# nikhilTkur/Multigrid_Nikhil_C-

Hardware: AMD Instinct MI355X
Metric: fine_grid_stencil_updates_per_sec (higher is better)
Workload: dtype f64

## Files before the change

### multigrid_nikhil_c-_amd/csrc/mgx.hip

```cpp

#include "../../include/mgx.h"
#include "mgx_bottom.hpp"
#include "mgx_kernels.hpp"
#include "mgx_launch.hpp"
#include "mgx_var.hpp"
#include "mgx_krylov.hpp"
#include "mgx_dist_plan.hpp"

#include <chrono>
#include <unistd.h>
#include <cmath>
#include <cstdio>
#include <cstdlib>
#include <cstring>
#include <string>
#include <vector>

namespace {

using namespace mgx;

thread_local std::string g_create_error;

void log_runtime_libs(const char* where)
// ... 181 lines not shown
void free_level(Level& l)
{
    for (void** p : {&l.u, &l.b, &l.tmp, &l.r, &l.coef[0], &l.coef[1], &l.coef[2], &l.coef[3], &l.coef[4],
                     &l.jac[0], &l.jac[1], &l.jac[2], &l.jac[3], &l.jac[4]}) {
        if (*p) (void)hipFree(*p);
        *p = nullptr;
    }
}

int ensure_r(mgx_solver* s, Level& l)
{
    if (l.r) return MGX_OK;
    if (hipMalloc(&l.r, l.bytes) != hipSuccess) return s->fail(MGX_ERR_ALLOC, "hipMalloc failed for residual array");
    HIPCHK(s, hipMemsetAsync(l.r, 0, l.bytes, s->stream));
    return MGX_OK;
}

bool level_ok(const mgx_solver* s, int level)
{
    return level >= s->cfg.coarsest_level && level <= s->cfg.finest_level;
}

int copy_in(mgx_solver* s, Level& l, void* dst_grid, const void* src, size_t count)
{
    const size_t n = (size_t)l.N - 1;
    if (count != n * n) return s->fail(MGX_ERR_INVALID, "vector length must be n*n with n = 2^level - 1");
    const size_t es = l.esize();
    char* d = reinterpret_cast<char*>(dst_grid) + ((size_t)l.pitch + 1) * es;
    HIPCHK(s, hipMemcpy2DAsync(d, (size_t)l.pitch * es, src, n * es, n * es, n, hipMemcpyHostToDevice, s->stream));
    HIPCHK(s, hipStreamSynchronize(s->stream));
    return MGX_OK;
}

int copy_out(mgx_solver* s, Level& l, const void* src_grid, void* dst, size_t count)
{
    const size_t n = (size_t)l.N - 1;
    if (count != n * n) return s->fail(MGX_ERR_INVALID, "vector length must be n*n with n = 2^level - 1");
    const size_t es = l.esize();
    const char* p = reinterpret_cast<const char*>(src_grid) + ((size_t)l.pitch + 1) * es;
    HIPCHK(s, hipMemcpy2DAsync(dst, n * es, p, (size_t)l.pitch * es, n * es, n, hipMemcpyDeviceToHost, s->stream));
    HIPCHK(s, hipStreamSynchronize(s->stream));
    return MGX_OK;
}

inline bool tile_level(const mgx_solver* s, const Level& l) { return s->fuse.tile_max_n > 0 && l.N <= s->fuse.tile_max_n; }

void smooth_t(mgx_solver* s, Level& l, int mu)
{
    with_kernel_set(l.f64, s->cfg.smoother, s->fuse.arith, [&](auto k) {
        using K = decltype(k);
        using T = typename K::T;
        int parity = 0, launches = 0;
        if (tile_level(s, l) && smooth_tiled<T, K::SM, K::AR>((T*)l.u, (const T*)l.b, (T*)l.tmp, l.N, l.pitch, mu, s->cfg.omega,
                                                              s->fuse.tile_k, FoldArgs(), false, 0, false, s->stream, &launches) >= 0)
            parity = launches & 1;
        else
            (void)smooth_block<T>(s->cfg.smoother, (T*)l.u, (const T*)l.b, (T*)l.tmp, l.N, l.pitch, l.rows, 1, l.N, mu,
                                  s->cfg.omega, false, 1, l.N, 0, s->rows_per_chunk, s->fuse, s->stream, &parity, &launches);
        s->last_smooth_launches = launches;
        if (parity) std::swap(l.u, l.tmp);
    });
}

int var_alloc_level(mgx_solver* s, Level& l)
{
    for (void** p : {&l.coef[0], &l.coef[1], &l.coef[2], &l.coef[3], &l.coef[4], &l.jac[0], &l.jac[1], &l.jac[2], &l.jac[3], &l.jac[4]}) {
        if (hipMalloc(p, l.bytes) != hipSuccess) return s->fail(MGX_ERR_ALLOC, "hipMalloc failed for the operator's coefficient arrays");
        HIPCHK(s, hipMemsetAsync(*p, 0, l.bytes, s->stream));
    }
    return MGX_OK;
}

template <typename T>
int var_build_t(mgx_solver* s, Level& l)
{
    const dim3 blk(256), grd((l.N + 1 + 255) / 256, l.N + 1);
    hipLaunchKernelGGL((k_var_build_jacobi<T>), grd, blk, 0, s->stream, (const T*)l.coef[0], (const T*)l.coef[1], (const T*)l.coef[2],
                       (const T*)l.coef[3], (const T*)l.coef[4], (T*)l.jac[0], (T*)l.jac[1], (T*)l.jac[2], (T*)l.jac[3], (T*)l.jac[4],
                       l.N, l.pitch, (T)s->cfg.omega);
    if (l.L == s->cfg.coarsest_level && s->cfg.bottom == MGX_BOTTOM_EXACT) {
        const int n = l.N - 1, NN = n * n;
        hipLaunchKernelGGL((k_var_dense_fill<T>), dim3((NN + 255) / 256, NN), dim3(256), 0, s->stream, s->var_M, s->var_inv,
                           (const T*)l.coef[0], (const T*)l.coef[1], (const T*)l.coef[2], (const T*)l.coef[3], (const T*)l.coef[4], n, l.pitch);
        for (int k = 0; k < NN; ++k) {
            hipLaunchKernelGGL(k_gj_prow, dim3((NN + 255) / 256), dim3(256), 0, s->stream, s->var_M, s->var_inv, s->var_pm, s->var_pi, NN, k);
            hipLaunchKernelGGL(k_gj_elim, dim3(NN), dim3(256), 0, s->stream, s->var_M, s->var_inv, s->var_pm, s->var_pi, NN, k);
        }
    }
    HIPCHK(s, hipGetLastError());
    HIPCHK(s, hipStreamSynchronize(s->stream));
    l.stencil_set = true;
    for (auto& g : s->graphs) if (g.exec) (void)hipGraphExecDestroy(g.exec);
    s->graphs.clear();
    return MGX_OK;
}
int var_build(mgx_solver* s, Level& l) { return l.f64 ? var_build_t<double>(s, l) : var_build_t<float>(s, l); }

int var_ready(mgx_solver* s, int lo, int hi)
{
    if (!s->var) return MGX_OK;
    for (int l = lo; l <= hi; ++l)
        if (!s->lv[l].stencil_set)
            return s->fail(MGX_ERR_STATE, "operator of level " + std::to_string(l) + " not set (mgx_set_stencil / mgx_set_coefficient)");
    return MGX_OK;
}

template <typename T>
// ... 64 lines not shown
    const int smax = std::max(1, kcap / per);
    std::vector<double> best(mu + 1, 1e300);
    std::vector<int> pick(mu + 1, 1);
    best[0] = 0.0;
    for (int m = 1; m <= mu; ++m)
        for (int k = 1; k <= std::min(m, smax); ++k) {
            const double c = fold_pass_cost(per * k, smoother, N, post, f64, f.arith);
            if (c < 0.0) continue;
            if (k == mu && m == mu && !cycle_k_supported(per * k, rbgs, f64, post, pre, f.arith)) continue;
            const double t = best[m - k] + c + 1e-3;
            if (t < best[m] - 1e-12) { best[m] = t; pick[m] = k; }
        }
    int n = 0;
    for (int m = mu; m > 0; m -= pick[m]) parts[n++] = pick[m];
    std::sort(parts, parts + n, [](int a, int b) { return a > b; });
    return n;
}

template <typename T, int SM, int AR>
int fold_block(const FuseCfg& fc, long tile_points, const mgx_slab* f, T* u, const T* b, T* tmp, int row_lo, int row_hi,
               int mu, double omega, const mgx_slab* c, const T* coarse_e, T* coarse_b, T* coarse_zero, int crow_lo,
               int crow_hi, int restrict_mode, int zero_in, int post, double* partial, hipStream_t st, int* flips)
{
    constexpr bool rbgs = (SM == 1);
    constexpr int per = rbgs ? 2 : 1;
    const bool pre = (coarse_e != nullptr);
    const int N = 1 << f->level;
    const long pitch = level_pitch(f->level, f->dtype);
    const int first = 1 - f->row0, last = N - f->row0;
    const JacobiCoef<T> jc = jacobi_coef<T>(omega);
    FoldArgs fa;
    fa.restrict_mode = restrict_mode;
    fa.partial = partial;
    fa.win.row_first = std::max(f->row0, 0);
    fa.win.row_last = std::min(f->row0 + f->rows - 1, N);
    fa.win.crow_first = 0; fa.win.crow_last = -1; fa.win.emit_lo = 0; fa.win.emit_hi = 0;
    if (c) {
        fa.cpitch = level_pitch(c->level, c->dtype);
        fa.win.crow_first = std::max(c->row0, 0);
        fa.win.crow_last = std::min(c->row0 + c->rows - 1, N / 2);
        fa.win.emit_lo = std::max(c->row0 + crow_lo, 1);
        fa.win.emit_hi = std::min(c->row0 + crow_hi, N / 2);
        const long cback = (long)c->row0 * fa.cpitch;
        if (coarse_e) fa.coarse_e = coarse_e - cback;
        if (coarse_b) fa.coarse_b = coarse_b - cback;
        if (coarse_zero) fa.coarse_zero = coarse_zero - cback;
    }
    const long back = (long)f->row0 * pitch;
    {
        const int lo = std::max(std::max(row_lo, first), 1), hi = std::min(std::min(row_hi, last), f->rows - 1);
        const bool whole = row_lo <= first && row_hi >= last;
        if (fc.tile_max_n > 0 && hi > lo && (long)(hi - lo) * N <= tile_points && (per * mu <= fc.tile_k || whole)) {
            fa.row_lo = lo + f->row0; fa.row_hi = hi + f->row0;
            return smooth_tiled<T, SM, AR>(u - back, b - back, tmp - back, N, pitch, mu, omega, fc.tile_k, fa, pre, post,
                                           zero_in != 0, st, flips);
        }
    }
    int parts[64];
    const int np = fold_plan(fc, rbgs ? MGX_SMOOTHER_RBGS : MGX_SMOOTHER_JACOBI, N, sizeof(T) == 8, mu, pre, post, parts);
    const int rpc = env_int("MGX_ROWS", 0);
    T* src = u; T* dst = tmp;
    int done = 0, blocks = 0;
    for (int p = 0; p < np; ++p) {
        const int sw = parts[p], K = per * sw;
        const bool P = pre && p == 0;
        const int Q = (p == np - 1) ? post : 0;
        fa.zero_in = (p == 0 && zero_in) ? 1 : 0;
        const int ext = per * (mu - (done + sw)) + (p != np - 1 ? (post == 2 ? 1 : (post == 1 ? 2 : 0)) : 0);
        const int lo = std::max(std::max(row_lo - ext, first), 1), hi = std::min(std::min(row_hi + ext, last), f->rows - 1);
        if (hi > lo) {
            const int R = fuse_rows(fc, N, K, sizeof(T) == 8, hi - lo);
            if (P || Q) {
                if (!cycle_k_supported(K, rbgs, sizeof(T) == 8, Q, P, AR)) return -1;
                fa.row_lo = lo + f->row0; fa.row_hi = hi + f->row0;
                const int Rc = fuse_rows_auto(fc, N, K, sizeof(T) == 8) ? -R : R;
                const int rc = with_stages(P, Q, [&](auto s) {
                    using S = decltype(s);
                    if constexpr (S::PRE || S::POST)
                        return launch_cycle<T, S::PRE, S::POST, SM, AR>(K, src - back, b - back, dst - back, fa, N, pitch, jc.c0, jc.c1, Rc, st);
                    else
                        return -1;
                });
                if (rc < 0) return -1;
                if (Q == 2) blocks = rc;
            } else if (!rbgs && K == 1) {
                if (fa.zero_in) return -1;
                if (launch_jacobi<T>(src, b, dst, N, pitch, lo, hi, omega, rpc, st, f->rows, AR)) return -1;
            } else if (!launch_fused<T, SM, AR>(K, src, b, dst, N, pitch, lo, hi, jc.c0, jc.c1, first - 1, last, f->row0 & 1, R, st, f->rows, fa.zero_in)) {
                return -1;
            }
        }
        std::swap(src, dst);
        done += sw;
    }
    *flips = np;
    return blocks;
}

bool fold_eligible(const mgx_solver* s, const Level& l, int mu, bool pre = false, int post = 1)
{
    if (!s->fold || mu < 1 || mu > 64) return false;
    if (s->var || (post == 1 && s->cfg.restrict_mode >= MGX_RESTRICT_INJECT)) return false;
    if (tile_level(s, l)) return true;
    if (l.N < s->fuse.min_n) return false;
    const bool rbgs = (s->cfg.smoother == MGX_SMOOTHER_RBGS);
    const int per = rbgs ? 2 : 1;
    if (s->fuse.kmax < per) return false;
    int parts[64];
// ... 1551 lines not shown
```

### multigrid_nikhil_c-_amd/csrc/mgx_geom.hpp

```cpp
#pragma once

#if defined(__HIPCC__)
#define MGX_GEOM_HD __host__ __device__ __forceinline__
#else
#define MGX_GEOM_HD inline
#endif

namespace mgx {

constexpr int kGeomWavesPerBlock = 4;
constexpr int kGeomCusPerXcd = 32;
constexpr int kGeomResidentBlocks = 512;

struct CycleGeom {
    int R, Re, Rl;
    int Rf;
    int chunks, chunks_e;
    int row_last0;
    int RB, n_tall, n_short;
    long waves;
    int blocks;
};

struct CTile { int strip, r0, r1; bool active; };
// ... 175 lines not shown
        const int mid = row_last0 - (row_lo + rf);
        if (mid < rb) continue;
        const int nt_max = (8 * slots - 7 - n_edge) / si, ns_max = (8 * slots - 7) / si;
        if (nt_max < 1 || ns_max < 1) continue;
        if ((long)nt_max * ra + (long)ns_max * rb < mid) continue;
        if (rb < kn.pair_min_rows) return false;
        int nt = (int)((double)mid * ((double)nt_max * ra / ((double)nt_max * ra + (double)ns_max * rb)) / ra + 0.5);
        if (nt > nt_max) nt = nt_max;
        while (nt > 0 && (long)nt * ra > mid - rb) --nt;
        int ns = nt > 0 ? (mid - nt * ra + rb - 1) / rb : ns_max + 1;
        while (ns > ns_max && nt < nt_max && (long)(nt + 1) * ra <= mid - rb) { ++nt; ns = (mid - nt * ra + rb - 1) / rb; }
        if (nt < 1 || ns > ns_max) continue;
        const int pf = (n_edge + nt * si + 7) / 8, ps = (ns * si + 7) / 8;
        if (pf > slots || ps > slots) continue;
        CycleGeom g;
        g.R = ra; g.Re = re; g.Rl = rl; g.Rf = rf; g.RB = rb; g.n_tall = nt; g.n_short = ns;
        g.chunks_e = chunks_e; g.row_last0 = row_last0; g.chunks = 3 + nt + ns;
        g.waves = (long)g.chunks * si + 2L * chunks_e;
        g.blocks = geom_blocks(g, strips);
        if (g.blocks > kGeomResidentBlocks) continue;
        *out = g;
        return true;
    }
    return false;
}

inline CycleGeom cycle_geom_pick(int row_lo, int row_hi, int strips, int extra, int trip, int R, bool auto_rows, bool deep,
                                 const GeomKnobs& kn, bool top_edge = true, bool bot_edge = true)
{
    if (R & 1) ++R;
    R = trip_rows(R, extra, trip, 2);
    CycleGeom g = cycle_geom(row_lo, row_hi, strips, R, R, R);
    if (!deep) return g;
    auto shaped = [&](int r) {
        return cycle_geom(row_lo, row_hi, strips, r, kn.edge_short ? edge_rows_pct(r, extra, trip, kn.edge_pct) : r,
                          (kn.edge_short && bot_edge) ? edge_rows_pct(r, extra, trip, kn.last_pct) : r,
                          (kn.edge_short && top_edge) ? edge_rows_pct(r, extra, trip, kn.edge_pct) : r);
    };
    if (!auto_rows) return kn.edge_short ? shaped(R) : g;
    if (kn.pair && kn.edge_short && strips >= 3) {
        CycleGeom p;
        if (cycle_geom_paired(row_lo, row_hi, strips, extra, trip, kn, top_edge, bot_edge, &p)) return p;
    }
    bool found = false;
    for (int m = (row_hi - row_lo >= kn.min_rounds_rows ? kn.min_rounds : 1); m <= 64 && !found; ++m) {
        for (int r = trip_rows(kn.min_chunk, extra, trip, 2); r <= 204; r += trip) {
            const CycleGeom c = shaped(r);
            if (c.waves <= 2048L * m && c.blocks <= kGeomResidentBlocks * m) { g = c; found = true; break; }
        }
    }
    return g;
}

}
```

### multigrid_nikhil_c-_amd/csrc/mgx_inst.hip

```cpp
#include "mgx_launch.hpp"

namespace mgx {
using T_ = MGX_INST_T;
#if MGX_INST_KIND == 1
#if MGX_INST_PP == 0
#define PP_ 1, 2
#elif MGX_INST_PP == 1
#define PP_ 1, 0
#elif MGX_INST_PP == 2
#define PP_ 0, 1
#elif MGX_INST_PP == 3
#define PP_ 0, 2
#else
#define PP_ 1, 1
#endif
template int launch_cycle<T_, PP_, MGX_INST_SM, MGX_INST_AR>(int, const T_*, const T_*, T_*, const FoldArgs&, int, long, T_, T_, int, hipStream_t);
#elif MGX_INST_KIND == 2
template bool launch_fused<T_, MGX_INST_SM, MGX_INST_AR>(int, const T_*, const T_*, T_*, int, long, int, int, T_, T_, int, int, int, int, hipStream_t, int, int);
#elif MGX_INST_KIND == 3
template int smooth_tiled<T_, MGX_INST_SM, MGX_INST_AR>(T_*, const T_*, T_*, int, long, int, double, int, FoldArgs, bool, int, bool, hipStream_t, int*);
#else
#error "MGX_INST_KIND must be 1, 2 or 3"
#endif
}
```

### multigrid_nikhil_c-_amd/csrc/mgx_kernels.hpp

```cpp
#pragma once

#include <hip/hip_runtime.h>
#include "mgx_geom.hpp"
#include <stdint.h>
#include <type_traits>

namespace mgx {

template <int B, int E, typename F> __device__ __forceinline__ void static_for(F&& f)
{
    if constexpr (B < E) {
        f(std::integral_constant<int, B>{});
        static_for<B + 1, E>(f);
    }
}

constexpr int kWave = 64;
constexpr int kBlock = 256;
constexpr int kWavesPerBlock = kBlock / kWave;
constexpr int kOutLanes = kWave - 2;

template <typename T> struct VecOf;
template <> struct VecOf<double> { using type = double2; static constexpr int W = 2; };
template <> struct VecOf<float>  { using type = float4;  static constexpr int W = 4; };
// ... 1400 lines not shown
        double acc = 0.0;
        T prev = up;
#pragma unroll
        for (int i = 0; i < RW; ++i) {
            const T cur = u[i];
            const T below = (i == RW - 1) ? dn : u[i + 1];
            const int y = y0 + i, gy = gy0 + i;
            const T l = from_left(cur), r = from_right(cur);
            T rr = (T)0;
            if (colunk && gy > 0 && gy < N) rr = b[i] - (-nbr(prev, l, r, below) + (T)4 * cur);
            res[i] = rr;
            if (POST == 2 && y >= He && y < He + TH && gy >= row_lo && gy < row_hi && colout) acc += (double)rr * (double)rr;
            prev = cur;
        }
        if (POST == 2) {
            for (int off = 32; off > 0; off >>= 1) acc += __shfl_down(acc, off, kWave);
            if (lane == 0) wsum[wv] = acc;
            __syncthreads();
            if (threadIdx.x == 0) {
                double sum = 0.0;
                for (int w2 = 0; w2 < kWavesPerBlock; ++w2) sum += wsum[w2];
                partial[blockIdx.x] = sum;
            }
        }
        if (POST == 1) {
            T rup, rdn;
            halo_rows(res, rup, rdn);
            const int J = gx >> 1;
            const bool cst = colout && (gx & 1) == 0 && J >= 1 && J < NC;
#pragma unroll
            for (int i = 0; i < RW; ++i) {
                const T c = res[i];
                const T n = (i == 0) ? rup : res[i - 1];
                const T s2 = (i == RW - 1) ? rdn : res[i + 1];
                const int y = y0 + i, gy = gy0 + i;
                T corners = from_left(n) + from_right(n);
                corners = corners + from_left(s2);
                corners = corners + from_right(s2);
                T edges = from_left(c) + from_right(c);
                edges = edges + n;
                edges = edges + s2;
                const T o = wgt * ((corners + (T)2 * edges) + (T)4 * c);
                if (cst && y >= He && y < He + TH && (gy & 1) == 0 && gy < N && gy >= row_lo && gy < row_hi &&
                    (gy >> 1) >= win.emit_lo && (gy >> 1) < win.emit_hi) {
                    const long at = (long)(gy >> 1) * cpitch + J;
                    coarse_b[at] = o;
                    if (coarse_zero) coarse_zero[at] = (T)0;
                }
            }
        }
    }
}

static __global__ void __launch_bounds__(kBlock)
k_axpy_f32_to_f64(double* __restrict__ u, const float* __restrict__ e, double scale, int N, long pitch, long epitch,
                  int row_lo, int row_hi, int R, int strips, int chunks, int assign)
{
    const Tile t = wave_tile(strips, chunks);
    if (!t.active) return;
    const Cols c = lane_cols<2>(t.strip, N, pitch);
    const int r0 = row_lo + t.chunk * R;
    const int r1 = min(r0 + R, row_hi);
    for (int r = r0; r < r1; ++r) {
        if (c.st) {
            const float2 ev = *reinterpret_cast<const float2*>(e + (long)r * epitch + c.col);
            double2* pu = reinterpret_cast<double2*>(u + (long)r * pitch + c.col);
            double2 o = assign ? make_double2(0.0, 0.0) : *pu;
            o.x = o.x + scale * (double)ev.x;
            o.y = o.y + scale * (double)ev.y;
            if (c.col == 0) o.x = 0.0;
            *pu = o;
        }
    }
}

static __global__ void __launch_bounds__(kBlock)
k_update_residual(const double* __restrict__ u, const float* __restrict__ e, const double* __restrict__ rhs,
                  double* __restrict__ unew, float* __restrict__ r32, double scale, double inv_scale,
                  double* __restrict__ partial, int N, long pitch, long epitch, int row_lo, int row_hi,
                  int R, int strips, int chunks)
{
    __shared__ double wsum[kWavesPerBlock];
    const Tile t = wave_tile(strips, chunks);
    double acc = 0.0;
    if (t.active) {
        const Cols c = lane_cols<2>(t.strip, N, pitch);
        const int r0 = row_lo + t.chunk * R;
        const int r1 = min(r0 + R, row_hi);
        auto updated = [&](int r) {
            double2 o = make_double2(0.0, 0.0);
            if (c.ld) {
                const double2 uv = *reinterpret_cast<const double2*>(u + (long)r * pitch + c.col);
                const float2 ev = *reinterpret_cast<const float2*>(e + (long)r * epitch + c.col);
                o.x = uv.x + scale * (double)ev.x;
                o.y = uv.y + scale * (double)ev.y;
                if (c.col == 0) o.x = 0.0;
            }
            return o;
        };
        double2 up = updated(r0 - 1);
        double2 cur = updated(r0);
        for (int r = r0; r < r1; ++r) {
            const double2 dn = updated(r + 1);
            const double2 bb = vload<double2>(rhs + (long)r * pitch + c.col, c.ld);
            double2 o = residual_vec(up, cur, dn, bb);
            mask_cols(o, c.col, N);
// ... 64 lines not shown
```

### multigrid_nikhil_c-_amd/csrc/mgx_launch.hpp

```cpp
#pragma once

#include "../../include/mgx.h"
#include "mgx_kernels.hpp"

#include <algorithm>
#include <cstdlib>
#include <vector>

namespace mgx {

inline long level_pitch(int level, int dtype)
{
    const long N = 1L << level;
    const long align = (dtype == MGX_DTYPE_F64) ? 32 : 64;
    return (N + 1 + align - 1) / align * align;
}

inline int env_int(const char* name, int dflt)
{
    const char* s = getenv(name);
    return (s && *s) ? atoi(s) : dflt;
}

struct FuseCfg {
    int kmax; int rows; int min_n; int fold_kmax; int fold_kmax_big; int tile_max_n; int tile_k; int fold_kmax_nopost;
    int plan_pre[8] = {0}; int n_pre = 0; int plan_post[8] = {0}; int n_post = 0; int plan_min_n = 8192;
    int arith = 0;
};

template <typename T> struct JacobiCoef { T c0, c1; };
template <typename T>
JacobiCoef<T> jacobi_coef(double omega)
{
    const T om = (T)omega;
    return {(T)(1.0 - (double)om), (T)((double)om / 4.0)};
}

template <typename T_, int SM_, int AR_> struct KernelSet { using T = T_; static constexpr int SM = SM_, AR = AR_; };
template <typename F>
decltype(auto) with_kernel_set(bool f64, int smoother, int arith, F&& f)
{
    const bool rbgs = (smoother == MGX_SMOOTHER_RBGS);
    if (f64) return rbgs ? f(KernelSet<double, 1, 0>{}) : (arith ? f(KernelSet<double, 0, 1>{}) : f(KernelSet<double, 0, 0>{}));
    return rbgs ? f(KernelSet<float, 1, 0>{}) : (arith ? f(KernelSet<float, 0, 1>{}) : f(KernelSet<float, 0, 0>{}));
}

template <typename T>
int launch_jacobi(const T* vin, const T* b, T* vout, int N, long pitch, int row_lo, int row_hi,
                  double omega, int rpc, hipStream_t st, int rows_alloc, int arith = 0)
{
    if (row_hi <= row_lo) return MGX_OK;
    if (row_lo < 1 || row_hi > rows_alloc - 1) return MGX_ERR_INVALID;
    const auto [c0, c1] = jacobi_coef<T>(omega);
    if (rpc <= 0) {
        const Launch g = make_launch(N, VecOf<T>::W, row_hi - row_lo, 1);
        if (arith) hipLaunchKernelGGL((k_jacobi_rows<T, 1>), dim3(g.blocks), dim3(kBlock), 0, st, vin, b, vout, N, pitch,
                                      row_lo, row_hi, g.strips, c0, c1, rows_alloc);
        else hipLaunchKernelGGL((k_jacobi_rows<T, 0>), dim3(g.blocks), dim3(kBlock), 0, st, vin, b, vout, N, pitch,
                                row_lo, row_hi, g.strips, c0, c1, rows_alloc);
        return MGX_OK;
    }
    const Launch g = make_launch(N, VecOf<T>::W, row_hi - row_lo, rpc);
    if (arith) hipLaunchKernelGGL((k_jacobi<T, 1>), dim3(g.blocks), dim3(kBlock), 0, st, vin, b, vout, N, pitch,
                                  row_lo, row_hi, g.R, g.strips, g.chunks, c0, c1, rows_alloc);
    else hipLaunchKernelGGL((k_jacobi<T, 0>), dim3(g.blocks), dim3(kBlock), 0, st, vin, b, vout, N, pitch,
                            row_lo, row_hi, g.R, g.strips, g.chunks, c0, c1, rows_alloc);
    return MGX_OK;
}

template <typename T>
void launch_rbgs(const T* vin, const T* b, T* vout, int N, long pitch, int row_lo, int row_hi,
                 int row_parity, int bnd_lo, int bnd_hi, int rpc, hipStream_t st)
{
    if (row_hi <= row_lo) return;
    const Launch g = make_launch(N, VecOf<T>::W, row_hi - row_lo, rpc);
    hipLaunchKernelGGL((k_rbgs<T>), dim3(g.blocks), dim3(kBlock), 0, st, vin, b, vout, N, pitch,
                       row_lo, row_hi, g.R, g.strips, g.chunks, row_parity, bnd_lo, bnd_hi);
}
// ... 32 lines not shown
        }
    }
    return false;
}

inline int fuse_rows_deep(int N, int rows)
{
    const int strips = (N / 2 + 51) / 52;
    const int cpr = std::max(1, 2048 / strips);
    for (int m = 1; m <= 64; ++m) {
        const int R = (rows + m * cpr - 1) / (m * cpr);
        if (R <= 200) return std::max(R, 16);
    }
    return 64;
}

inline bool fuse_rows_auto(const FuseCfg& fc, int N, int K, bool f64)
{
    return fc.rows <= 0 && K >= (f64 ? 8 : 10) && N >= 2048;
}

inline int shallow_big_n() { static const int n = env_int("MGX_SHALLOW_BIG_N", 8192); return n; }
inline int shallow_mid_rows() { static const int r = env_int("MGX_SHALLOW_ROWS_MID", 48); return r; }

inline int fuse_rows(const FuseCfg& fc, int N, int K, bool f64 = true, int rows = 0)
{
    if (fc.rows > 0) return fc.rows;
    if (K <= 2) {
        static const int big2 = env_int("MGX_SHALLOW2_ROWS_BIG", 96);
        return N >= shallow_big_n() ? big2 : (N >= 4096 ? shallow_mid_rows() : 8);
    }
    if (K <= 4) {
        static const int big = env_int("MGX_SHALLOW_ROWS_BIG", 96);
        return N >= shallow_big_n() ? big : (N >= 4096 ? shallow_mid_rows() : 16);
    }
    if (f64 && K >= 8 && N >= 2048) return fuse_rows_deep(N, rows > 0 ? rows : N - 1);
    int R = N / 128;
    if (R < 8) R = 8;
    if (R > (f64 ? 64 : 32)) R = f64 ? 64 : 32;
    return R;
}

inline FuseCfg fuse_cfg()
{
    FuseCfg f;
    f.kmax = env_int("MGX_FUSE", 10);
    if (f.kmax < 1) f.kmax = 1;
    if (f.kmax > 10) f.kmax = 10;
    f.rows = env_int("MGX_FUSE_ROWS", 0);
    if (f.rows < 0) f.rows = 0;
    f.min_n = std::max(64, env_int("MGX_FUSE_MIN_N", 256));
    f.fold_kmax = std::max(1, std::min(f.kmax, env_int("MGX_FOLD_KMAX", 10)));
    f.fold_kmax_big = std::max(1, std::min(f.kmax, env_int("MGX_FOLD_KMAX_BIG", 10)));
    f.tile_max_n = std::max(0, env_int("MGX_TILE_MAX_N", 1024));
    f.tile_k = std::max(2, std::min(10, env_int("MGX_TILE_K", 10)));
    f.fold_kmax_nopost = std::max(1, std::min(f.kmax, env_int("MGX_FOLD_KMAX_NOPOST", 10)));
    auto parse = [](const char* name, int* out) {
        const char* v = std::getenv(name);
        int n = 0;
        while (v && *v && n < 8) {
            char* end = nullptr;
            const long k = std::strtol(v, &end, 10);
            if (end == v || k < 1 || k > 10) return 0;
            out[n++] = (int)k;
            v = (*end == ',') ? end + 1 : end;
            if (*end && *end != ',') return 0;
        }
        return n;
    };
    f.n_pre = parse("MGX_PLAN_PRE", f.plan_pre);
    f.n_post = parse("MGX_PLAN_POST", f.plan_post);
    f.plan_min_n = env_int("MGX_PLAN_MIN_N", 8192);
    return f;
}

constexpr double kFuseRate64[11] = {0, 1.00, 1.80, 2.45, 3.16, 3.81, 4.80, 0, 5.60, 0, 5.63};
constexpr double kFuseRate32[11] = {0, 1.00, 1.67, 2.38, 3.10, 3.77, 4.26, 0, 4.98, 0, 4.67};
constexpr double kFuseRateGS64[11] = {0, 1.00, 1.81, 2.50, 3.19, 3.12, 0, 0, 0, 0, 0};
constexpr double kFuseRateGS32[11] = {0, 1.00, 1.79, 2.20, 2.87, 2.69, 0, 0, 0, 0, 0};

inline int plan_fusion(int mu, int kmax, bool f64, int* parts, bool rbgs = false)
{
    const double* rate = rbgs ? (f64 ? kFuseRateGS64 : kFuseRateGS32) : (f64 ? kFuseRate64 : kFuseRate32);
    const int per = rbgs ? 2 : 1;
    const int smax = std::max(1, std::min(kmax, 10) / per);
    std::vector<double> best(mu + 1, 1e300);
    std::vector<int> pick(mu + 1, 1);
    best[0] = 0.0;
    for (int m = 1; m <= mu; ++m)
        for (int k = 1; k <= std::min(m, smax); ++k) {
            if (rate[k] <= 0.0) continue;
            const double c = best[m - k] + (double)k / rate[k] + 0.02;
            if (c < best[m]) { best[m] = c; pick[m] = k; }
        }
    int n = 0;
    for (int m = mu; m > 0; m -= pick[m]) parts[n++] = pick[m];
    return n;
}

template <typename T>
int smooth_block(int smoother, T* a, const T* rhs, T* b2, int N, long pitch, int rows_alloc, int row_lo, int row_hi,
                 int mu, double omega, bool shrink, int first, int last, int row_parity, int rpc, const FuseCfg& fc,
                 hipStream_t st, int* parity, int* launches = nullptr)
{
    const bool rbgs = (smoother == MGX_SMOOTHER_RBGS);
    const int per = rbgs ? 2 : 1;
// ... 103 lines not shown
    }
    if constexpr (sizeof(T) == 8 || PRE == 1 || POST == 0) {
        if (K == 8) return launch_cycle_k<T, 8, PRE, POST, SM, AR>(vin, b, vout, fa, N, pitch, c0, c1, R, st);
    }
    if constexpr (!(PRE == 1 && POST == 1) && !(SM == 1 && POST == 1) && !(sizeof(T) == 4 && PRE == 1 && POST == 2) &&
                  !(sizeof(T) == 4 && POST == 1 && AR == 0)) {
        if (K == 10) return launch_cycle_k<T, 10, PRE, POST, SM, AR>(vin, b, vout, fa, N, pitch, c0, c1, R, st);
    }
    if constexpr (SM == 0) {
        switch (K) {
            case 1: return launch_cycle_k<T, 1, PRE, POST, 0, AR>(vin, b, vout, fa, N, pitch, c0, c1, R, st);
            case 3: return launch_cycle_k<T, 3, PRE, POST, 0, AR>(vin, b, vout, fa, N, pitch, c0, c1, R, st);
            case 5: return launch_cycle_k<T, 5, PRE, POST, 0, AR>(vin, b, vout, fa, N, pitch, c0, c1, R, st);
            default: break;
        }
    }
    return -1;
}

inline bool cycle_k_supported(int K, bool rbgs, bool f64, int post, bool pre, int arith)
{
    if (K == 10) return !(pre && post == 1) && !(rbgs && post == 1) && !(!f64 && pre && post == 2) && !(!f64 && post == 1 && arith == 0);
    if (K == 8 && !f64 && !pre && post != 0) return false;
    return rbgs ? (K == 2 || K == 4 || K == 6 || K == 8) : (K >= 1 && K <= 8 && K != 7);
}

template <int PRE_, int POST_> struct Stages { static constexpr int PRE = PRE_, POST = POST_; };
template <typename F>
int with_stages(bool pre, int post, F&& f)
{
    if (pre) return post == 2 ? f(Stages<1, 2>{}) : (post == 1 ? f(Stages<1, 1>{}) : f(Stages<1, 0>{}));
    return post == 2 ? f(Stages<0, 2>{}) : (post == 1 ? f(Stages<0, 1>{}) : f(Stages<0, 0>{}));
}

template <typename T, int SM, int PRE, int POST, int AR>
int launch_tile(const T* vin, const T* b, T* vout, const FoldArgs& fa, int N, long pitch, T c0, T c1, int levels,
                hipStream_t st)
{
    const int He = levels + tile_extra<POST>();
    const int TH = kTileSY - 2 * He, TW = kTileSX - 2 * He;
    if (TH < 8 || TW < 8) return -1;
    const bool whole = (fa.row_hi == 0);
    const int row_lo = whole ? 1 : fa.row_lo, row_hi = whole ? N : fa.row_hi;
    const CycleWin win = whole ? CycleWin{0, N, 0, N / 2, 1, N / 2} : fa.win;
    const int tiles_y = (row_hi - row_lo + TH - 1) / TH, tiles_x = (N - 1 + TW - 1) / TW;
    if (tiles_y < 1) return 0;
    const T w = (fa.restrict_mode == MGX_RESTRICT_FW16) ? (T)0.0625 : (T)0.25;
    hipLaunchKernelGGL((k_tile_smooth<T, SM, PRE, POST, AR>), dim3(tiles_y * tiles_x), dim3(kBlock), 0, st, vin, b, vout,
                       (const T*)fa.coarse_e, (T*)fa.coarse_b, (T*)fa.coarse_zero, w, fa.partial, N, pitch, fa.cpitch,
                       levels, c0, c1, tiles_x, fa.zero_in, row_lo, row_hi, win);
    return tiles_y * tiles_x;
}

template <typename T, int SM, int AR>
int smooth_tiled(T* a, const T* rhs, T* b2, int N, long pitch, int mu, double omega, int tile_k, FoldArgs fa,
                 bool pre, int post, bool zero_in, hipStream_t st, int* flips)
{
    constexpr int per = (SM == 1) ? 2 : 1;
    const JacobiCoef<T> jc = jacobi_coef<T>(omega);
    const int smax = std::max(1, tile_k / per);
    const int np = (mu + smax - 1) / smax;
    T* src = a; T* dst = b2;
    int blocks = 0;
    for (int p = 0; p < np; ++p) {
        const int sw = mu / np + (p < mu % np ? 1 : 0);
        const bool P = pre && p == 0;
        const int Q = (p == np - 1) ? post : 0;
        fa.zero_in = (p == 0 && zero_in) ? 1 : 0;
        const int rc = with_stages(P, Q, [&](auto s) {
            return launch_tile<T, SM, decltype(s)::PRE, decltype(s)::POST, AR>(src, rhs, dst, fa, N, pitch, jc.c0, jc.c1, per * sw, st);
        });
        if (rc < 0) return -1;
        if (Q == 2) blocks = rc;
        std::swap(src, dst);
    }
    *flips = np;
    return blocks;
}

template <typename T>
void launch_restrict(const T* v, const T* b, T* cb, T* czero, int N, long pitch, long cpitch,
                     int crow_lo, int crow_hi, int fine_row_off, int mode, bool fused, int rpc, hipStream_t st)
{
    if (crow_hi <= crow_lo) return;
    Launch g = make_launch(N, VecOf<T>::W, crow_hi - crow_lo, rpc > 0 ? (rpc + 1) / 2 : 0);
    const T w = (mode == MGX_RESTRICT_FW16) ? (T)0.0625 : (T)0.25;
    if (fused)
        hipLaunchKernelGGL((k_restrict<T, true>), dim3(g.blocks), dim3(kBlock), 0, st, v, b, cb, czero, N, pitch,
                           cpitch, crow_lo, crow_hi, fine_row_off, g.R, g.strips, g.chunks, w);
    else
        hipLaunchKernelGGL((k_restrict<T, false>), dim3(g.blocks), dim3(kBlock), 0, st, v, b, cb, czero, N, pitch,
                           cpitch, crow_lo, crow_hi, fine_row_off, g.R, g.strips, g.chunks, w);
}

template <typename T>
void launch_prolong(T* v, const T* e, int N, long pitch, long cpitch, int row_lo, int row_hi,
                    int fine_row_off, bool add, int rpc, hipStream_t st)
{
    if (row_hi <= row_lo) return;
    const Launch g = make_launch(N, VecOf<T>::W, row_hi - row_lo, rpc);
    if (add)
        hipLaunchKernelGGL((k_prolong<T, true>), dim3(g.blocks), dim3(kBlock), 0, st, v, e, N, pitch, cpitch,
                           row_lo, row_hi, fine_row_off, g.R, g.strips, g.chunks);
    else
        hipLaunchKernelGGL((k_prolong<T, false>), dim3(g.blocks), dim3(kBlock), 0, st, v, e, N, pitch, cpitch,
                           row_lo, row_hi, fine_row_off, g.R, g.strips, g.chunks);
}

template <typename T> long sumsq_blocks(int N, int rows, int rpc)
{
    return make_launch(N, VecOf<T>::W, rows, rpc).blocks;
}

template <typename T, int MODE>
void launch_residual(const T* v, const T* b, void* out, long pitch_out, double* partial, double* sum_dev,
                     double inv_scale, int N, long pitch, int row_lo, int row_hi, int rpc, hipStream_t st,
                     long partial_cap, int rows_alloc)
{
    Launch g = make_launch(N, VecOf<T>::W, row_hi - row_lo, rpc);
    if (MODE != 0 && partial_cap >= 0 && g.blocks > partial_cap) {
        const int R = (int)(((long)g.strips * (row_hi - row_lo) / kWavesPerBlock + partial_cap - 9) / (partial_cap - 8)) + 1;
        g = make_launch(N, VecOf<T>::W, row_hi - row_lo, R);
    }
    hipLaunchKernelGGL((k_residual<T, MODE>), dim3(g.blocks), dim3(kBlock), 0, st, v, b, out, pitch_out, partial,
                       inv_scale, N, pitch, row_lo, row_hi, g.R, g.strips, g.chunks, rows_alloc);
    if (MODE != 0)
        hipLaunchKernelGGL(k_reduce_partials, dim3(1), dim3(kReduceThreads), 0, st, partial, g.blocks, sum_dev);
}


#define MGX_FOR_SMAR(X, T) X(T, 0, 0) X(T, 0, 1) X(T, 1, 0)
#define MGX_DECL_CYCLE_PP(T, PRE, POST, SM, AR) \
    extern template int launch_cycle<T, PRE, POST, SM, AR>(int, const T*, const T*, T*, const FoldArgs&, int, long, T, T, int, hipStream_t);
#define MGX_DECL_CYCLE(T, SM, AR) MGX_DECL_CYCLE_PP(T, 1, 2, SM, AR) MGX_DECL_CYCLE_PP(T, 1, 0, SM, AR) MGX_DECL_CYCLE_PP(T, 0, 1, SM, AR) \
    MGX_DECL_CYCLE_PP(T, 0, 2, SM, AR) MGX_DECL_CYCLE_PP(T, 1, 1, SM, AR)
#define MGX_DECL_FUSED(T, SM, AR) \
    extern template bool launch_fused<T, SM, AR>(int, const T*, const T*, T*, int, long, int, int, T, T, int, int, int, int, hipStream_t, int, int);
#define MGX_DECL_TILE(T, SM, AR) \
    extern template int smooth_tiled<T, SM, AR>(T*, const T*, T*, int, long, int, double, int, FoldArgs, bool, int, bool, hipStream_t, int*);
#if !defined(MGX_INST_KIND) && !defined(MGX_SINGLE_TU)
MGX_FOR_SMAR(MGX_DECL_CYCLE, double) MGX_FOR_SMAR(MGX_DECL_CYCLE, float)
MGX_FOR_SMAR(MGX_DECL_FUSED, double) MGX_FOR_SMAR(MGX_DECL_FUSED, float)
MGX_FOR_SMAR(MGX_DECL_TILE, double) MGX_FOR_SMAR(MGX_DECL_TILE, float)
#endif

}
```

Before: 1070 billion.

## Add wide-tile temporal-blocked smoother kernel with register row bands per wave

Adds a new k_tile_wide kernel for tiled levels. Each 8-wave block holds a band of 8 or 10 rows per wave in registers, and halo rows are exchanged between waves through double-buffered shared memory. The prolongation correction, the residual and the restriction are fused in as before. By default it runs for f64 on levels up to N=1024, aiming to cut per-tile halo recomputation and global traffic compared with the older tile kernel. The cost is more registers per thread, which may lower occupancy, plus more halo overlap per tile.

Measured after the change: 1086 billion (median of 6 runs). 1.02x the previous value.

```diff
diff --git a/multigrid_nikhil_c-_amd/csrc/mgx.hip b/multigrid_nikhil_c-_amd/csrc/mgx.hip
--- a/multigrid_nikhil_c-_amd/csrc/mgx.hip
+++ b/multigrid_nikhil_c-_amd/csrc/mgx.hip
@@ -257,7 +257,8 @@
         using T = typename K::T;
         int parity = 0, launches = 0;
         if (tile_level(s, l) && smooth_tiled<T, K::SM, K::AR>((T*)l.u, (const T*)l.b, (T*)l.tmp, l.N, l.pitch, mu, s->cfg.omega,
-                                                              s->fuse.tile_k, FoldArgs(), false, 0, false, s->stream, &launches) >= 0)
+                                                              s->fuse.tile_k, tile_band<T>(s->fuse, l.N), FoldArgs(), false, 0, false,
+                                                              s->stream, &launches) >= 0)
             parity = launches & 1;
         else
             (void)smooth_block<T>(s->cfg.smoother, (T*)l.u, (const T*)l.b, (T*)l.tmp, l.N, l.pitch, l.rows, 1, l.N, mu,
@@ -428,8 +429,8 @@
         const bool whole = row_lo <= first && row_hi >= last;
         if (fc.tile_max_n > 0 && hi > lo && (long)(hi - lo) * N <= tile_points && (per * mu <= fc.tile_k || whole)) {
             fa.row_lo = lo + f->row0; fa.row_hi = hi + f->row0;
-            return smooth_tiled<T, SM, AR>(u - back, b - back, tmp - back, N, pitch, mu, omega, fc.tile_k, fa, pre, post,
-                                           zero_in != 0, st, flips);
+            return smooth_tiled<T, SM, AR>(u - back, b - back, tmp - back, N, pitch, mu, omega, fc.tile_k, tile_band<T>(fc, N), fa,
+                                           pre, post, zero_in != 0, st, flips);
         }
     }
     int parts[64];
diff --git a/multigrid_nikhil_c-_amd/csrc/mgx_geom.hpp b/multigrid_nikhil_c-_amd/csrc/mgx_geom.hpp
--- a/multigrid_nikhil_c-_amd/csrc/mgx_geom.hpp
+++ b/multigrid_nikhil_c-_amd/csrc/mgx_geom.hpp
@@ -251,4 +251,26 @@
     return g;
 }
 
-}
+constexpr int kTileWideWaves = 8;
+
+struct TileWideGeom {
+    int He, Hx;
+    int TH, TW;
+    int tiles_y, tiles_x;
+};
+
+MGX_GEOM_HD TileWideGeom tile_wide_geom(int N, int row_lo, int row_hi, int He, int W, int RW)
+{
+    TileWideGeom g;
+    g.He = He;
+    g.Hx = (He + W - 1) / W * W;
+    g.TH = kTileWideWaves * RW - 2 * He;
+    g.TW = 64 * W - 2 * g.Hx;
+    g.tiles_y = (g.TH > 0 && row_hi > row_lo) ? (row_hi - row_lo + g.TH - 1) / g.TH : 0;
+    g.tiles_x = g.TW > 0 ? (N + g.TW - 1) / g.TW : 0;
+    return g;
+}
+
+MGX_GEOM_HD int tile_wide_rw(int N, int short_max_n) { return N <= short_max_n ? 8 : 10; }
+
+}
diff --git a/multigrid_nikhil_c-_amd/csrc/mgx_inst.hip b/multigrid_nikhil_c-_amd/csrc/mgx_inst.hip
--- a/multigrid_nikhil_c-_amd/csrc/mgx_inst.hip
+++ b/multigrid_nikhil_c-_amd/csrc/mgx_inst.hip
@@ -18,7 +18,7 @@
 #elif MGX_INST_KIND == 2
 template bool launch_fused<T_, MGX_INST_SM, MGX_INST_AR>(int, const T_*, const T_*, T_*, int, long, int, int, T_, T_, int, int, int, int, hipStream_t, int, int);
 #elif MGX_INST_KIND == 3
-template int smooth_tiled<T_, MGX_INST_SM, MGX_INST_AR>(T_*, const T_*, T_*, int, long, int, double, int, FoldArgs, bool, int, bool, hipStream_t, int*);
+template int smooth_tiled<T_, MGX_INST_SM, MGX_INST_AR>(T_*, const T_*, T_*, int, long, int, double, int, int, FoldArgs, bool, int, bool, hipStream_t, int*);
 #else
 #error "MGX_INST_KIND must be 1, 2 or 3"
 #endif
diff --git a/multigrid_nikhil_c-_amd/csrc/mgx_kernels.hpp b/multigrid_nikhil_c-_amd/csrc/mgx_kernels.hpp
--- a/multigrid_nikhil_c-_amd/csrc/mgx_kernels.hpp
+++ b/multigrid_nikhil_c-_amd/csrc/mgx_kernels.hpp
@@ -1476,6 +1476,221 @@
     }
 }
 
+__device__ __forceinline__ double vget(const double2& v, int e) { return e == 0 ? v.x : v.y; }
+__device__ __forceinline__ float vget(const float4& v, int e) { return e == 0 ? v.x : (e == 1 ? v.y : (e == 2 ? v.z : v.w)); }
+__device__ __forceinline__ double2 vmake(const double (&a)[2]) { return make_double2(a[0], a[1]); }
+__device__ __forceinline__ float4 vmake(const float (&a)[4]) { return make_float4(a[0], a[1], a[2], a[3]); }
+
+template <typename T, int SM, int PRE, int POST, int AR, int RW>
+__global__ void __launch_bounds__(kTileWideWaves * kWave)
+k_tile_wide(const T* __restrict__ vin, const T* __restrict__ rhs, T* __restrict__ vout,
+            const T* __restrict__ coarse_e, T* __restrict__ coarse_b, T* __restrict__ coarse_zero, T wgt,
+            double* __restrict__ partial, int N, long pitch, long cpitch, int levels, T c0, T c1,
+            int tiles_x, int zero_in, int row_lo, int row_hi, CycleWin win)
+{
+    using V = typename VecOf<T>::type;
+    constexpr int W = VecOf<T>::W;
+    constexpr int NW = kTileWideWaves;
+    __shared__ V edge[2][NW][2][kWave];
+    __shared__ double wsum[NW];
+    const TileWideGeom g = tile_wide_geom(N, row_lo, row_hi, levels + tile_extra<POST>(), W, RW);
+    const int He = g.He, TH = g.TH, TW = g.TW;
+    const int lane = threadIdx.x & 63;
+    const int wv = __builtin_amdgcn_readfirstlane(threadIdx.x >> 6);
+    const int ty = blockIdx.x / tiles_x, tx = blockIdx.x - ty * tiles_x;
+    const int y0 = wv * RW;
+    const int gy0 = row_lo + ty * TH - He + y0;
+    const int cx0 = tx * TW;
+    const int gx0 = cx0 - g.Hx + W * lane;
+    const bool vld = gx0 >= 0 && gx0 < N;
+    const bool cu0 = vld && gx0 > 0;
+    bool cu[W];
+#pragma unroll
+    for (int e = 0; e < W; ++e) cu[e] = e == 0 ? cu0 : vld;
+    const int NC = N / 2;
+
+    T u[RW][W], b[RW][W];
+    unsigned rowmask = 0;
+#pragma unroll
+    for (int i = 0; i < RW; ++i) {
+        const int gy = gy0 + i;
+        const bool rowok = gy > 0 && gy < N && gy >= win.row_first && gy <= win.row_last;
+        if (rowok) rowmask |= 1u << i;
+        const long at = (long)gy * pitch + gx0;
+        V uv = vzero((V*)nullptr), bv = vzero((V*)nullptr);
+        if (vld && rowok) {
+            bv = *reinterpret_cast<const V*>(rhs + at);
+            if (!zero_in) uv = *reinterpret_cast<const V*>(vin + at);
+        }
+#pragma unroll
+        for (int e = 0; e < W; ++e) {
+            u[i][e] = cu[e] ? vget(uv, e) : (T)0;
+            b[i][e] = cu[e] ? vget(bv, e) : (T)0;
+        }
+    }
+    if (PRE) {
+        constexpr int NCR = RW / 2 + 1, NCC = W / 2 + 1;
+        const int kc0 = gy0 >> 1, J = gx0 >> 1;
+        T cr[NCR][NCC];
+#pragma unroll
+        for (int k = 0; k < NCR; ++k) {
+            const int cy = kc0 + k;
+            const bool ok = vld && cy >= 0 && cy <= NC && cy >= win.crow_first && cy <= win.crow_last;
+            const T* ep = coarse_e + (long)cy * cpitch + J;
+#pragma unroll
+            for (int m = 0; m < NCC; ++m) cr[k][m] = ok ? ep[m] : (T)0;
+        }
+        auto correct = [&](auto parity) {
+            constexpr int par = decltype(parity)::value;
+#pragma unroll
+            for (int i = 0; i < RW; ++i) {
+                const int gy = gy0 + i;
+                const bool rodd = ((par + i) & 1) != 0;
+                const int kr = (par + i) >> 1;
+                const bool rin = ((rowmask >> i) & 1u) && (gy >> 1) >= win.crow_first && (gy >> 1) + (rodd ? 1 : 0) <= win.crow_last;
+#pragma unroll
+                for (int e = 0; e < W; ++e) {
+                    const bool codd = (e & 1) != 0;
+                    const bool unk = cu[e] && rin;
+                    const T a00 = unk ? cr[kr][e >> 1] : (T)0;
+                    const T a01 = (unk && codd) ? cr[kr][(e >> 1) + 1] : (T)0;
+                    const T a10 = (unk && rodd) ? cr[kr + (rodd ? 1 : 0)][e >> 1] : (T)0;
+                    const T a11 = (unk && rodd && codd) ? cr[kr + (rodd ? 1 : 0)][(e >> 1) + 1] : (T)0;
+                    const T ev = codd ? (T)0.5 * (a00 + a01) : a00;
+                    const T od = codd ? (T)0.25 * (((a00 + a10) + a01) + a11) : (T)0.5 * (a00 + a10);
+                    const T add = rodd ? od : ev;
+                    u[i][e] = unk ? u[i][e] + add : u[i][e];
+                }
+            }
+        };
+        if (gy0 & 1) correct(std::integral_constant<int, 1>{});
+        else correct(std::integral_constant<int, 0>{});
+    }
+
+    int buf = 0;
+    auto halo_rows = [&](const T (&a)[RW][W], T (&up)[W], T (&dn)[W]) {
+        edge[buf][wv][0][lane] = vmake(a[0]);
+        edge[buf][wv][1][lane] = vmake(a[RW - 1]);
+        __syncthreads();
+        const V uv = wv > 0 ? edge[buf][wv - 1][1][lane] : vzero((V*)nullptr);
+        const V dv = wv < NW - 1 ? edge[buf][wv + 1][0][lane] : vzero((V*)nullptr);
+#pragma unroll
+        for (int e = 0; e < W; ++e) { up[e] = vget(uv, e); dn[e] = vget(dv, e); }
+        buf ^= 1;
+    };
+    for (int j = 1; j <= levels; ++j) {
+        T up[W], dn[W];
+        halo_rows(u, up, dn);
+        const int colour = (j - 1) & 1;
+        T prev[W];
+#pragma unroll
+        for (int e = 0; e < W; ++e) prev[e] = up[e];
+#pragma unroll
+        for (int i = 0; i < RW; ++i) {
+            T cur[W];
+#pragma unroll
+            for (int e = 0; e < W; ++e) cur[e] = u[i][e];
+            const T l = from_left(cur[W - 1]), r = from_right(cur[0]);
+            const bool rowact = (rowmask >> i) & 1u;
+#pragma unroll
+            for (int e = 0; e < W; ++e) {
+                const T below = (i == RW - 1) ? dn[e] : u[i + 1][e];
+                const T we = e == 0 ? l : cur[e - 1], ea = e == W - 1 ? r : cur[e + 1];
+                if (SM == 0) {
+                    const T o = jac_pt<AR>(c0, cur[e], c1 * b[i][e], c1, nbr(prev[e], we, ea, below));
+                    u[i][e] = (cu[e] && rowact) ? o : cur[e];
+                } else {
+                    const T o = (T)0.25 * (b[i][e] + nbr(prev[e], we, ea, below));
+                    u[i][e] = (cu[e] && rowact && ((gy0 + i + e) & 1) == colour) ? o : cur[e];
+                }
+            }
+#pragma unroll
+            for (int e = 0; e < W; ++e) prev[e] = cur[e];
+        }
+    }
+
+    const bool colout = gx0 >= cx0 && gx0 < cx0 + TW && gx0 < N;
+#pragma unroll
+    for (int i = 0; i < RW; ++i) {
+        const int y = y0 + i, gy = gy0 + i;
+        if (y >= He && y < He + TH && gy < N && gy >= row_lo && gy < row_hi && colout)
+            *reinterpret_cast<V*>(vout + (long)gy * pitch + gx0) = vmake(u[i]);
+    }
+
+    if (POST != 0) {
+        T up[W], dn[W];
+        halo_rows(u, up, dn);
+        T res[RW][W];
+        double acc = 0.0;
+        T prev[W];
+#pragma unroll
+        for (int e = 0; e < W; ++e) prev[e] = up[e];
+#pragma unroll
+        for (int i = 0; i < RW; ++i) {
+            const int y = y0 + i, gy = gy0 + i;
+            const T l = from_left(u[i][W - 1]), r = from_right(u[i][0]);
+            const bool rowunk = gy > 0 && gy < N;
+            const bool rowout = POST == 2 && y >= He && y < He + TH && gy >= row_lo && gy < row_hi && colout;
+#pragma unroll
+            for (int e = 0; e < W; ++e) {
+                const T cur = u[i][e];
+                const T below = (i == RW - 1) ? dn[e] : u[i + 1][e];
+                const T we = e == 0 ? l : u[i][e - 1], ea = e == W - 1 ? r : u[i][e + 1];
+                T rr = (T)0;
+                if (cu[e] && rowunk) rr = b[i][e] - (-nbr(prev[e], we, ea, below) + (T)4 * cur);
+                res[i][e] = rr;
+                if (rowout) acc += (double)rr * (double)rr;
+            }
+#pragma unroll
+            for (int e = 0; e < W; ++e) prev[e] = u[i][e];
+        }
+        if (POST == 2) {
+            for (int off = 32; off > 0; off >>= 1) acc += __shfl_down(acc, off, kWave);
+            if (lane == 0) wsum[wv] = acc;
+            __syncthreads();
+            if (threadIdx.x == 0) {
+                double sum = 0.0;
+                for (int w2 = 0; w2 < NW; ++w2) sum += wsum[w2];
+                partial[blockIdx.x] = sum;
+            }
+        }
+        if (POST == 1) {
+            T rup[W], rdn[W];
+            halo_rows(res, rup, rdn);
+#pragma unroll
+            for (int i = 0; i < RW; ++i) {
+                const int y = y0 + i, gy = gy0 + i;
+                const bool rowst = y >= He && y < He + TH && (gy & 1) == 0 && gy < N && gy >= row_lo && gy < row_hi &&
+                                   (gy >> 1) >= win.emit_lo && (gy >> 1) < win.emit_hi;
+                T n[W], s2[W];
+#pragma unroll
+                for (int e = 0; e < W; ++e) {
+                    n[e] = (i == 0) ? rup[e] : res[i - 1][e];
+                    s2[e] = (i == RW - 1) ? rdn[e] : res[i + 1][e];
+                }
+                const T nl = from_left(n[W - 1]), sl = from_left(s2[W - 1]), cl = from_left(res[i][W - 1]);
+#pragma unroll
+                for (int e = 0; e < W; e += 2) {
+                    const T c = res[i][e];
+                    T corners = (e == 0 ? nl : n[e - 1]) + n[e + 1];
+                    corners = corners + (e == 0 ? sl : s2[e - 1]);
+                    corners = corners + s2[e + 1];
+                    T edges = (e == 0 ? cl : res[i][e - 1]) + res[i][e + 1];
+                    edges = edges + n[e];
+                    edges = edges + s2[e];
+                    const T o = wgt * ((corners + (T)2 * edges) + (T)4 * c);
+                    const int J = (gx0 + e) >> 1;
+                    if (rowst && colout && J >= 1 && J < NC) {
+                        const long at = (long)(gy >> 1) * cpitch + J;
+                        coarse_b[at] = o;
+                        if (coarse_zero) coarse_zero[at] = (T)0;
+                    }
+                }
+            }
+        }
+    }
+}
+
 static __global__ void __launch_bounds__(kBlock)
 k_axpy_f32_to_f64(double* __restrict__ u, const float* __restrict__ e, double scale, int N, long pitch, long epitch,
                   int row_lo, int row_hi, int R, int strips, int chunks, int assign)
diff --git a/multigrid_nikhil_c-_amd/csrc/mgx_launch.hpp b/multigrid_nikhil_c-_amd/csrc/mgx_launch.hpp
--- a/multigrid_nikhil_c-_amd/csrc/mgx_launch.hpp
+++ b/multigrid_nikhil_c-_amd/csrc/mgx_launch.hpp
@@ -24,6 +24,7 @@
 
 struct FuseCfg {
     int kmax; int rows; int min_n; int fold_kmax; int fold_kmax_big; int tile_max_n; int tile_k; int fold_kmax_nopost;
+    int tile_wide; int tile_short_n;
     int plan_pre[8] = {0}; int n_pre = 0; int plan_post[8] = {0}; int n_post = 0; int plan_min_n = 8192;
     int arith = 0;
 };
@@ -162,6 +163,8 @@
     f.min_n = std::max(64, env_int("MGX_FUSE_MIN_N", 256));
     f.fold_kmax = std::max(1, std::min(f.kmax, env_int("MGX_FOLD_KMAX", 10)));
     f.fold_kmax_big = std::max(1, std::min(f.kmax, env_int("MGX_FOLD_KMAX_BIG", 10)));
+    f.tile_wide = std::max(0, std::min(2, env_int("MGX_TILE_WIDE", 1)));
+    f.tile_short_n = env_int("MGX_TILE_SHORT_N", 512);
     f.tile_max_n = std::max(0, env_int("MGX_TILE_MAX_N", 1024));
     f.tile_k = std::max(2, std::min(10, env_int("MGX_TILE_K", 10)));
     f.fold_kmax_nopost = std::max(1, std::min(f.kmax, env_int("MGX_FOLD_KMAX_NOPOST", 10)));
@@ -371,8 +374,41 @@
     return tiles_y * tiles_x;
 }
 
+template <typename T, int SM, int PRE, int POST, int AR>
+int launch_tile_wide(const T* vin, const T* b, T* vout, const FoldArgs& fa, int N, long pitch, T c0, T c1, int levels,
+                     int rw, hipStream_t st)
+{
+    if (VecOf<T>::W == 4) rw = 8;
+    const bool whole = (fa.row_hi == 0);
+    const int row_lo = whole ? 1 : fa.row_lo, row_hi = whole ? N : fa.row_hi;
+    const CycleWin win = whole ? CycleWin{0, N, 0, N / 2, 1, N / 2} : fa.win;
+    const TileWideGeom g = tile_wide_geom(N, row_lo, row_hi, levels + tile_extra<POST>(), VecOf<T>::W, rw);
+    if (g.TH < 8 || g.TW < 8) return -1;
+    if (g.tiles_y < 1) return 0;
+    const T w = (fa.restrict_mode == MGX_RESTRICT_FW16) ? (T)0.0625 : (T)0.25;
+    const dim3 grid(g.tiles_y * g.tiles_x), block(kTileWideWaves * kWave);
+    if (rw == 8)
+        hipLaunchKernelGGL((k_tile_wide<T, SM, PRE, POST, AR, 8>), grid, block, 0, st, vin, b, vout, (const T*)fa.coarse_e,
+                           (T*)fa.coarse_b, (T*)fa.coarse_zero, w, fa.partial, N, pitch, fa.cpitch, levels, c0, c1, g.tiles_x,
+                           fa.zero_in, row_lo, row_hi, win);
+    else if constexpr (VecOf<T>::W == 2) {
+        if (rw != 10) return -1;
+        hipLaunchKernelGGL((k_tile_wide<T, SM, PRE, POST, AR, 10>), grid, block, 0, st, vin, b, vout, (const T*)fa.coarse_e,
+                           (T*)fa.coarse_b, (T*)fa.coarse_zero, w, fa.partial, N, pitch, fa.cpitch, levels, c0, c1, g.tiles_x,
+                           fa.zero_in, row_lo, row_hi, win);
+    } else {
+        return -1;
+    }
+    return g.tiles_y * g.tiles_x;
+}
+
+template <typename T> int tile_band(const FuseCfg& fc, int N)
+{
+    return (fc.tile_wide >= (sizeof(T) == 8 ? 1 : 2)) ? tile_wide_rw(N, fc.tile_short_n) : 0;
+}
+
 template <typename T, int SM, int AR>
-int smooth_tiled(T* a, const T* rhs, T* b2, int N, long pitch, int mu, double omega, int tile_k, FoldArgs fa,
+int smooth_tiled(T* a, const T* rhs, T* b2, int N, long pitch, int mu, double omega, int tile_k, int band, FoldArgs fa,
                  bool pre, int post, bool zero_in, hipStream_t st, int* flips)
 {
     constexpr int per = (SM == 1) ? 2 : 1;
@@ -387,7 +423,9 @@
         const int Q = (p == np - 1) ? post : 0;
         fa.zero_in = (p == 0 && zero_in) ? 1 : 0;
         const int rc = with_stages(P, Q, [&](auto s) {
-            return launch_tile<T, SM, decltype(s)::PRE, decltype(s)::POST, AR>(src, rhs, dst, fa, N, pitch, jc.c0, jc.c1, per * sw, st);
+            using S = decltype(s);
+            return band ? launch_tile_wide<T, SM, S::PRE, S::POST, AR>(src, rhs, dst, fa, N, pitch, jc.c0, jc.c1, per * sw, band, st)
+                        : launch_tile<T, SM, S::PRE, S::POST, AR>(src, rhs, dst, fa, N, pitch, jc.c0, jc.c1, per * sw, st);
         });
         if (rc < 0) return -1;
         if (Q == 2) blocks = rc;
@@ -456,7 +494,7 @@
 #define MGX_DECL_FUSED(T, SM, AR) \
     extern template bool launch_fused<T, SM, AR>(int, const T*, const T*, T*, int, long, int, int, T, T, int, int, int, int, hipStream_t, int, int);
 #define MGX_DECL_TILE(T, SM, AR) \
-    extern template int smooth_tiled<T, SM, AR>(T*, const T*, T*, int, long, int, double, int, FoldArgs, bool, int, bool, hipStream_t, int*);
+    extern template int smooth_tiled<T, SM, AR>(T*, const T*, T*, int, long, int, double, int, int, FoldArgs, bool, int, bool, hipStream_t, int*);
 #if !defined(MGX_INST_KIND) && !defined(MGX_SINGLE_TU)
 MGX_FOR_SMAR(MGX_DECL_CYCLE, double) MGX_FOR_SMAR(MGX_DECL_CYCLE, float)
 MGX_FOR_SMAR(MGX_DECL_FUSED, double) MGX_FOR_SMAR(MGX_DECL_FUSED, float)
```
